# astra-vision/SceneRF

Hardware: NVIDIA H100
Metric: rays/sec (higher is better)
Workload: dtype fp32 (2 x fp16 split operands, fp32 accumulate)

## Files before the change

### scenerf_b200/csrc/mlp_tc.cu

```cuda
#include <cuda.h>
#include <cuda_fp16.h>
#include <cstdio>
#include <cstdlib>
#include <cstring>
#include <type_traits>
#include "kernels.cuh"
#include "wgmma.cuh"

namespace srf {
namespace tc {

constexpr int kTileM = 64;
constexpr int kChunkK = 64;
constexpr int kAChunkBytes = kTileM * 128;
constexpr int kBRows = 128, kBSlotBytes = kBRows * 128;
constexpr int kHiddenChunks = kHidden / kChunkK;
constexpr int kQuarters = kHidden / kBRows;
constexpr int kOutN = 16;
constexpr int kOutImgBytes = kOutN * 128;
constexpr int kThreads = 256;
constexpr int kNumBias = 8;
constexpr size_t kHeaderBytes = (size_t)kNumBias * kHidden * sizeof(float);
constexpr int kNumLayers = 11;
constexpr int kScaleSlot = 7 * kHidden + 256, kInvScaleSlot = 7 * kHidden + 257;
constexpr size_t kScratchFloats = (size_t)2 * kTileM * kHidden;
constexpr size_t kExchangeOffset = (size_t)2 * 2 * 64 * 128;

constexpr int kSmemAct = 0;
constexpr int kSmemX = kSmemAct + kHiddenChunks * kAChunkBytes;
constexpr int kSmemZ = kSmemX + kAChunkBytes;
constexpr int kRingBytes = 4 * kBSlotBytes;
constexpr int kSmemRing = kSmemZ + 2 * kAChunkBytes;
constexpr int kSmemBar = kSmemRing + 2 * kRingBytes;
constexpr int kSmemSph = kSmemBar + 2 * 4 * 8;
constexpr int kSmemMask = kSmemSph + kTileM * 4;
constexpr int kSmemTotal = kSmemMask + 16;
static_assert(kSmemTotal + 1024 <= 232448, "shared memory budget");

struct Layer { int chunks_is_kz, chunks, fresh, signal, is_out; };
__constant__ Layer kLayers[kNumLayers] = {
    {0, 1, 1, 0, 0}, {1, 0, 0, 1, 0},
    {0, 8, 1, 1, 0}, {0, 8, 1, 0, 0}, {1, 0, 0, 1, 0},
    {0, 8, 1, 1, 0}, {0, 8, 1, 0, 0}, {1, 0, 0, 1, 0},
    {0, 8, 1, 1, 0}, {0, 8, 1, 1, 0},
    {0, 8, 1, 1, 1}};

struct KernelArgs {
  const float* pts;
  const float* viewdir;
  int n, n_per, n_tiles, kz;
  const unsigned char* wblob;
  float* scratch;
  float* raw_out;
  int d_out;
  int32_t* dbg_sphere;
  int skip_zero;
  int hidden_fp16;
  const unsigned char* preproj;
  int pre_W1, pre_H1;
  int debug_layer;
  float* debug_acc;
  int* error_flag;
};

__device__ __forceinline__ uint32_t smem_u32(const void* p) { return (uint32_t)__cvta_generic_to_shared(p); }

__device__ __forceinline__ void mbar_init(uint32_t bar, uint32_t count) {
  asm volatile("mbarrier.init.shared::cta.b64 [%0], %1;" ::"r"(bar), "r"(count) : "memory");
}
__device__ __forceinline__ void mbar_arrive_expect_tx(uint32_t bar, uint32_t bytes) {
  asm volatile("mbarrier.arrive.expect_tx.shared::cta.b64 _, [%0], %1;" ::"r"(bar), "r"(bytes) : "memory");
}
__device__ __forceinline__ bool mbar_try_wait(uint32_t bar, uint32_t parity) {
  uint32_t ok;
  asm volatile(
      "{\n\t.reg .pred p;\n\t"
      "mbarrier.try_wait.parity.shared::cta.b64 p, [%1], %2;\n\t"
      "selp.u32 %0, 1, 0, p;\n\t}"
      : "=r"(ok)
      : "r"(bar), "r"(parity)
      : "memory");
  return ok != 0;
}
__device__ __noinline__ void mbar_timeout(int* error_flag, uint32_t bar, uint32_t parity) {
  if (error_flag) atomicExch(error_flag, (int)(0x40000000u | ((bar & 0xFFFFF) << 4) | (parity & 1) | ((threadIdx.x >> 5) << 24)));
  __threadfence_system();
  __trap();
}
__device__ __noinline__ void mbar_wait_spin(uint32_t bar, uint32_t parity, int* error_flag) {
  const long long t0 = clock64();
  while (!mbar_try_wait(bar, parity)) {
    if (clock64() - t0 > 4000000000LL) mbar_timeout(error_flag, bar, parity);
  }
}
__device__ __forceinline__ void mbar_wait(uint32_t bar, uint32_t parity, int* error_flag) {
  if (mbar_try_wait(bar, parity)) return;
  mbar_wait_spin(bar, parity, error_flag);
}
__device__ __forceinline__ void fence_barrier_init() { asm volatile("fence.mbarrier_init.release.cluster;" ::: "memory"); }
__device__ __forceinline__ void fence_proxy_async_smem() { asm volatile("fence.proxy.async.shared::cta;" ::: "memory"); }

__device__ __forceinline__ uint64_t l2_policy_evict_last() {
  uint64_t pol;
  asm volatile("createpolicy.fractional.L2::evict_last.b64 %0, 1.0;" : "=l"(pol));
  return pol;
}
__device__ __forceinline__ void bulk_g2s(uint32_t dst_smem, const void* src, uint32_t bytes, uint32_t bar, uint64_t policy) {
  asm volatile("cp.async.bulk.shared::cluster.global.mbarrier::complete_tx::bytes.L2::cache_hint [%0], [%1], %2, [%3], %4;"
               ::"r"(dst_smem), "l"(src), "r"(bytes), "r"(bar), "l"(policy)
               : "memory");
}
__device__ __forceinline__ void named_bar_sync(int id, int threads) {
  asm volatile("bar.sync %0, %1;" ::"r"(id), "r"(threads) : "memory");
}
__device__ __forceinline__ void sts128(uint32_t addr, uint32_t a, uint32_t b, uint32_t c, uint32_t d) {
  asm volatile("st.shared.v4.b32 [%0], {%1, %2, %3, %4};" ::"r"(addr), "r"(a), "r"(b), "r"(c), "r"(d) : "memory");
}
__device__ __forceinline__ void sts32(uint32_t addr, uint32_t a) {
  asm volatile("st.shared.b32 [%0], %1;" ::"r"(addr), "r"(a) : "memory");
}
__device__ __forceinline__ uint32_t pack_relu_half2(float lo, float hi) {
  uint32_t d;
  asm("cvt.rn.relu.f16x2.f32 %0, %1, %2;" : "=r"(d) : "f"(hi), "f"(lo));
  return d;
}
__device__ __forceinline__ uint32_t pack_half2(float lo, float hi) {
  __half2 h = __floats2half2_rn(lo, hi);
  return *reinterpret_cast<uint32_t*>(&h);
}
__device__ __forceinline__ void split_half2(float a, float b, uint32_t& hi, uint32_t& lo) {
  const __half2 h = __floats2half2_rn(a, b);
  const float2 hf = __half22float2(h);
  const __half2 l = __floats2half2_rn(a - hf.x, b - hf.y);
  hi = *reinterpret_cast<const uint32_t*>(&h);
  lo = *reinterpret_cast<const uint32_t*>(&l);
}

__device__ __forceinline__ uint32_t sw128_offset(int row, int g) { return (uint32_t)(row * 128 + ((g ^ (row & 7)) << 4)); }

__device__ __forceinline__ int layer_chunks(int l, int kz) { return kLayers[l].chunks_is_kz ? kz : kLayers[l].chunks; }
__device__ __forceinline__ bool chunk_active(int l, int c, uint64_t mask) { return !kLayers[l].chunks_is_kz || ((mask >> c) & 1ull); }

__device__ __forceinline__ uint64_t chunk_mask_for_scales(const DevParams& p, uint32_t scale_bits, int kz) {
  uint64_t m = 0;
  for (int c = 0; c < kz; ++c) {
    const int lo = c * kChunkK, hi = lo + kChunkK;
    for (int s = 0; s < kScales; ++s)
      if (((scale_bits >> s) & 1u) && p.ch_off[s] < hi && p.ch_off[s + 1] > lo) m |= 1ull << c;
  }
  return m;
}

__device__ __forceinline__ size_t chunk_image_offset(int l, int k, int kz, int parts) {
  size_t off = 0;
  for (int i = 0; i < l; ++i) off += (size_t)layer_chunks(i, kz) * (kLayers[i].is_out ? kOutImgBytes : kQuarters * kBSlotBytes);
  return (off + (size_t)k * (kLayers[l].is_out ? kOutImgBytes : kQuarters * kBSlotBytes)) * (size_t)parts;
}

struct Cursor {
  int l = 0, k = 0, j = 0;
  __device__ __forceinline__ bool normalize(int kz, uint64_t mask, int last_layer, int wg) {
    while (l <= last_layer) {
      if (l == kNumLayers - 1 && wg != 0) return false;
      if (j >= (kLayers[l].is_out ? 1 : 2)) { j = 0; ++k; }
      if (k >= layer_chunks(l, kz)) { k = 0; ++l; continue; }
      if (!chunk_active(l, k, mask)) { ++k; continue; }
      return true;
    }
    return false;
  }
};

__device__ __forceinline__ int next_active(int kz, uint64_t mask, int c) {
  for (++c; c < kz; ++c)
    if ((mask >> c) & 1ull) return c;
  return -1;
}

template <bool H16, bool SPLIT, bool PRE>
__global__ void __launch_bounds__(kThreads, 1)
point_mlp_tc_kernel(const __grid_constant__ DevParams p, const __grid_constant__ KernelArgs a) {
  extern __shared__ __align__(1024) unsigned char smem_dyn[];
  unsigned char* smem = smem_dyn + ((1024u - (smem_u32(smem_dyn) & 1023u)) & 1023u);
  const uint32_t smem_base = smem_u32(smem);
  const int tid = threadIdx.x;
  const int wg = tid >> 7, t = tid & 127, w = t >> 5, lane = tid & 31;
  constexpr int kParts = SPLIT ? 2 : 1;
  constexpr int kPts = SPLIT ? kTileM / 2 : kTileM;
  constexpr int kSlotBytes = kBSlotBytes * kParts;
  constexpr int kSlots = kRingBytes / kSlotBytes;
  const uint32_t ring = smem_base + kSmemRing + (uint32_t)wg * kRingBytes;
  auto full_bar = [&](int s) { return smem_base + kSmemBar + 8u * (uint32_t)(wg * 4 + s); };
  short2* sph_smem = reinterpret_cast<short2*>(smem + kSmemSph);
  volatile unsigned long long* mask_smem = reinterpret_cast<volatile unsigned long long*>(smem + kSmemMask);

  if (tid == 0) {
    for (int s = 0; s < 8; ++s) mbar_init(smem_base + kSmemBar + 8u * s, 1);
    fence_barrier_init();
  }
  __syncthreads();

  const int kz = a.kz;
  const int last_layer = (a.debug_layer >= 0) ? a.debug_layer : (kNumLayers - 1);
  const unsigned char* images = a.wblob + kHeaderBytes;
  const float* bias = reinterpret_cast<const float*>(a.wblob);
  float* scratch = a.scratch + (size_t)blockIdx.x * kScratchFloats;
  float* hbuf = scratch + (size_t)wg * (2 * 64 * 128);
  float* xbuf = scratch + kExchangeOffset + (size_t)wg * (2 * 64 * 64);
  const uint64_t policy = l2_policy_evict_last();

  Cursor pc;
  bool p_live = false;
  uint32_t ppos = 0, cpos = 0, done = 0;
  uint64_t mask = 0;
  auto produce = [&]() {
    if (t != 0) return;
    while (p_live && ppos < done + (uint32_t)kSlots) {
      const bool is_out = kLayers[pc.l].is_out != 0;
      const unsigned char* src = images + chunk_image_offset(pc.l, pc.k, kz, kParts) + (is_out ? 0 : (size_t)(2 * wg + pc.j) * kSlotBytes);
      const uint32_t bytes = is_out ? (uint32_t)(kOutImgBytes * kParts) : (uint32_t)kSlotBytes;
      const int s = (int)(ppos % kSlots);
      mbar_arrive_expect_tx(full_bar(s), bytes);
      bulk_g2s(ring + (uint32_t)s * kSlotBytes, src, bytes, full_bar(s), policy);
      ++ppos;
      ++pc.j;
      p_live = pc.normalize(kz, mask, last_layer, wg);
    }
  };
  float acc0[64], acc1[64], acco[8];
  auto wait_slot = [&]() -> uint32_t {
    const int s = (int)(cpos % kSlots);
    mbar_wait(full_bar(s), (cpos / kSlots) & 1u, a.error_flag);
    return ring + (uint32_t)s * kSlotBytes;
  };
  auto release1 = [&]() {
    gmma::wait<1>();
    done = cpos - 1;
    produce();
  };
  auto mma_pair = [&](uint32_t a_addr, bool fresh) {
    const uint64_t ad = gmma::desc_sw128(a_addr);
    {
      const uint32_t b = wait_slot();
      gmma::fence();
#pragma unroll
      for (int k = 0; k < 4; ++k)
#pragma unroll
        for (int part = 0; part < kParts; ++part)
          gmma::mma_f16_n128(acc0, ad + 2 * k, gmma::desc_sw128(b + part * kBSlotBytes) + 2 * k, (fresh && k == 0 && part == 0) ? 0 : 1);
      gmma::commit();
      ++cpos;
    }
    release1();
    {
      const uint32_t b = wait_slot();
      gmma::fence();
#pragma unroll
      for (int k = 0; k < 4; ++k)
#pragma unroll
        for (int part = 0; part < kParts; ++part)
          gmma::mma_f16_n128(acc1, ad + 2 * k, gmma::desc_sw128(b + part * kBSlotBytes) + 2 * k, (fresh && k == 0 && part == 0) ? 0 : 1);
      gmma::commit();
      ++cpos;
    }
  };
  auto mma_out = [&](uint32_t a_addr, bool fresh) {
    const uint64_t ad = gmma::desc_sw128(a_addr);
    const uint32_t b = wait_slot();
    gmma::fence();
#pragma unroll
    for (int k = 0; k < 4; ++k)
#pragma unroll
      for (int part = 0; part < kParts; ++part)
        gmma::mma_f16_n16(acco, ad + 2 * k, gmma::desc_sw128(b + part * kOutImgBytes) + 2 * k, (fresh && k == 0 && part == 0) ? 0 : 1);
    gmma::commit();
    ++cpos;
  };
  auto retire1 = release1;
  auto retire0 = [&]() {
    gmma::wait<0>();
    gmma::fence_regs(acc0); gmma::fence_regs(acc1); gmma::fence_regs(acco);
    done = cpos;
    produce();
  };
  auto sync_all = [&]() { named_bar_sync(1, kThreads); };

  const short2* sph_cur = sph_smem;
  const int erow0 = 16 * w + (lane >> 2);
  const int ecol = 2 * (lane & 3);

  for (int tile = blockIdx.x; tile < a.n_tiles; tile += gridDim.x) {
    const int row0 = tile * kPts;
    if (tid == 0) mask_smem[0] = 0ull;
    sync_all();
    {
      uint32_t my_scales = 0;
      if (tid < kPts) {
        const int gi = row0 + tid;
        int sx = kSphereInvalid, sy = kSphereInvalid;
        if (gi < a.n) {
          point_to_sphere(p, a.pts[(size_t)gi * 3 + 0], a.pts[(size_t)gi * 3 + 1], a.pts[(size_t)gi * 3 + 2], sx, sy);
          if (a.dbg_sphere) { a.dbg_sphere[(size_t)gi * 2 + 0] = sx; a.dbg_sphere[(size_t)gi * 2 + 1] = sy; }
        }
        sph_smem[tid] = make_short2((short)max(min(sx, 32767), -32768), (short)max(min(sy, 32767), -32768));
        if (a.skip_zero) {
#pragma unroll
          for (int s = 0; s < kScales; ++s) my_scales |= scale_taps(p, s, sx, sy).any ? (1u << s) : 0u;
        }
      }
      if (a.skip_zero && tid < ((kPts + 31) & ~31)) {
        const uint32_t wbits = __reduce_or_sync(0xffffffffu, my_scales);
        if (lane == 0) {
          const unsigned long long bits = chunk_mask_for_scales(p, wbits, kz);
          if (bits) atomicOr((unsigned long long*)mask_smem, bits);
        }
      }
    }
    sync_all();
    mask = PRE ? 0ull : (a.skip_zero ? mask_smem[0] : ~0ull);
    pc = Cursor();
    p_live = pc.normalize(kz, mask, last_layer, wg);
    produce();

    const unsigned char* pre_row[2] = {nullptr, nullptr};
    if constexpr (PRE) {
#pragma unroll
      for (int hh = 0; hh < 2; ++hh) {
        const short2 sp = sph_cur[(erow0 + 8 * hh) % kPts];
        const bool in = sp.x >= 0 && sp.x < a.pre_W1 && sp.y >= 0 && sp.y < a.pre_H1;
        const size_t ridx = in ? (size_t)sp.y * a.pre_W1 + sp.x : (size_t)a.pre_W1 * a.pre_H1;
        pre_row[hh] = a.preproj + ridx * (size_t)(SRF_NUM_BLOCKS * kHidden * (SPLIT ? 4 : 2));
      }
    }

    if (tid < 2 * kPts) {
      const bool first = tid < kPts;
      const int xrow = first ? tid : tid - kPts;
      const int gi = row0 + xrow;
      const uint32_t slot_addr = smem_base + kSmemX;
      float qx = 0.f, qy = 0.f, qz = 0.f;
      if (gi < a.n) { qx = a.pts[(size_t)gi * 3 + 0]; qy = a.pts[(size_t)gi * 3 + 1]; qz = a.pts[(size_t)gi * 3 + 2]; }
      const float kPi = 3.14159274101257324f, kHalfPi = 1.57079637050628662f;
      auto sel3 = [](int i, float v0, float v1, float v2) { return i == 0 ? v0 : (i == 1 ? v1 : v2); };
      auto xval = [&](int idx, const float* vd) -> float {
        if (gi >= a.n) return 0.0f;
        if (idx < 3) return sel3(idx, qx, qy, qz);
        if (idx < 3 + 36) {
          const int j = idx - 3, fp = j / 3, cc = j - 3 * fp;
          float arg = fmul(sel3(cc, qx, qy, qz), kPi * (float)(1 << (fp >> 1)));
          if (fp & 1) arg = fadd(kHalfPi, arg);
          return sinf(arg);
        }
        if (idx < kDX) return sel3(idx - 39, vd[0], vd[1], vd[2]);
        return 0.0f;
      };
      float vd[3] = {0.f, 0.f, 0.f};
      if (!first && gi < a.n) {
        const float* vp = a.viewdir + (size_t)(gi / a.n_per) * 3;
        vd[0] = vp[0]; vd[1] = vp[1]; vd[2] = vp[2];
      }
      const int g_end = first ? 3 : 8;
#pragma unroll 1
      for (int g = first ? 0 : 3; g < g_end; ++g) {
        float v[8];
#pragma unroll
        for (int j = 0; j < 8; ++j) v[j] = xval(8 * g + j, vd);
        if constexpr (SPLIT) {
          uint32_t hi[4], lo[4];
#pragma unroll
          for (int j = 0; j < 4; ++j) split_half2(v[2 * j], v[2 * j + 1], hi[j], lo[j]);
          sts128(slot_addr + sw128_offset(xrow, g), hi[0], hi[1], hi[2], hi[3]);
          sts128(slot_addr + sw128_offset(xrow + kPts, g), lo[0], lo[1], lo[2], lo[3]);
        } else {
          sts128(slot_addr + sw128_offset(xrow, g), pack_half2(v[0], v[1]), pack_half2(v[2], v[3]), pack_half2(v[4], v[5]),
                 pack_half2(v[6], v[7]));
        }
      }
    }
    fence_proxy_async_smem();
    sync_all();

    constexpr int kItems = kPts / 32;
    int cur_scale = -1;
    int t_off[kItems];
    uint32_t t_ok[kItems];
    float t_w[kItems], t_n[kItems];
    int dxo = 0, dyo = 0;
    auto gather = [&](int c, uint32_t zaddr) {
      const int g = tid & 7;
      const int ch = c * kChunkK + g * 8;
      auto emit_vals = [&](int row, const float (&v)[8]) {
        if constexpr (SPLIT) {
          uint32_t hi[4], lo[4];
#pragma unroll
          for (int j = 0; j < 4; ++j) split_half2(v[2 * j], v[2 * j + 1], hi[j], lo[j]);
          sts128(zaddr + sw128_offset(row, g), hi[0], hi[1], hi[2], hi[3]);
          sts128(zaddr + sw128_offset(row + kPts, g), lo[0], lo[1], lo[2], lo[3]);
        } else {
          sts128(zaddr + sw128_offset(row, g), pack_half2(v[0], v[1]), pack_half2(v[2], v[3]), pack_half2(v[4], v[5]), pack_half2(v[6], v[7]));
        }
      };
      int s = -1;
#pragma unroll
      for (int i = 0; i < kScales; ++i)
        if (ch >= p.ch_off[i] && ch < p.ch_off[i + 1]) s = i;
      if (s >= 0 && s != cur_scale) {
        dxo = p.C[s]; dyo = p.W[s] * p.C[s];
#pragma unroll
        for (int i = 0; i < kItems; ++i) {
          const short2 sp16 = sph_cur[(tid >> 3) + 32 * i];
          const Taps tp = scale_taps(p, s, sp16.x, sp16.y);
          t_ok[i] = (tp.off[0] >= 0 ? 1u : 0u) | (tp.off[1] >= 0 ? 2u : 0u) | (tp.off[2] >= 0 ? 4u : 0u) | (tp.off[3] >= 0 ? 8u : 0u);
          int o0 = 0;
          if (tp.off[0] >= 0) o0 = tp.off[0];
          else if (tp.off[1] >= 0) o0 = tp.off[1] - dxo;
          else if (tp.off[2] >= 0) o0 = tp.off[2] - dyo;
          else if (tp.off[3] >= 0) o0 = tp.off[3] - dxo - dyo;
          t_off[i] = o0;
          t_w[i] = tp.fx; t_n[i] = tp.fy;
        }
        cur_scale = s;
      }
      const char* fbytes = (s >= 0) ? reinterpret_cast<const char*>(p.feat[s]) : nullptr;
      const int ch_in = (s >= 0) ? ch - p.ch_off[s] : 0;
      const bool f16 = p.feat_fp16 != 0;
#pragma unroll
      for (int u = 0; u < kItems; ++u) {
        const int row = (tid >> 3) + 32 * u;
        float acc[8];
        const uint32_t ok = (s >= 0) ? t_ok[u] : 0u;
        if (!ok) {
#pragma unroll
          for (int e = 0; e < 8; ++e) acc[e] = 0.0f;
          emit_vals(row, acc);
          continue;
        }
        const float wx = t_w[u], ny = t_n[u];
        const float e_ = fsub(1.0f, wx), so = fsub(1.0f, ny);
        const float tw4[4] = {fmul(so, e_), fmul(so, wx), fmul(ny, e_), fmul(ny, wx)};
        float v[4][8];
#pragma unroll
        for (int tp = 0; tp < 4; ++tp) {
          if ((ok >> tp) & 1u) {
            const size_t eidx = (size_t)(ch_in + t_off[u] + (tp & 1) * dxo + (tp >> 1) * dyo);
            if (f16) {
              const uint4 raw = __ldg(reinterpret_cast<const uint4*>(fbytes + eidx * 2));
              const uint32_t rw[4] = {raw.x, raw.y, raw.z, raw.w};
#pragma unroll
              for (int q = 0; q < 4; ++q) {
                const float2 f = __half22float2(*reinterpret_cast<const __half2*>(&rw[q]));
                v[tp][2 * q] = f.x; v[tp][2 * q + 1] = f.y;
              }
            } else {
              const float4* src = reinterpret_cast<const float4*>(fbytes + eidx * 4);
              const float4 a0 = __ldg(src), a1 = __ldg(src + 1);
              v[tp][0] = a0.x; v[tp][1] = a0.y; v[tp][2] = a0.z; v[tp][3] = a0.w;
              v[tp][4] = a1.x; v[tp][5] = a1.y; v[tp][6] = a1.z; v[tp][7] = a1.w;
            }
          } else {
#pragma unroll
            for (int e = 0; e < 8; ++e) v[tp][e] = 0.0f;
          }
        }
#pragma unroll
        for (int e = 0; e < 8; ++e) {
          acc[e] = fmul(v[0][e], tw4[0]);
#pragma unroll
          for (int tp = 1; tp < 4; ++tp) acc[e] = fadd(acc[e], fmul(v[tp][e], tw4[tp]));
        }
        emit_vals(row, acc);
      }
    };
    auto zpass = [&]() {
      cur_scale = -1;
      int c = next_active(kz, mask, -1);
      if (c < 0) return;
      gather(c, smem_base + kSmemZ);
      fence_proxy_async_smem();
      sync_all();
      for (int zi = 0; c >= 0; ++zi) {
        const int cn = next_active(kz, mask, c);
        mma_pair(smem_base + kSmemZ + (uint32_t)(zi & 1) * kAChunkBytes, false);
        if (cn >= 0) gather(cn, smem_base + kSmemZ + (uint32_t)((zi + 1) & 1) * kAChunkBytes);
        retire0();
        fence_proxy_async_smem();
        sync_all();
        c = cn;
      }
    };

    auto epilogue = [&](auto use_h_c, auto write_h_c, auto use_p_c, int bias_idx) __attribute__((always_inline)) {
      constexpr bool USE_H = decltype(use_h_c)::value, WRITE_H = decltype(write_h_c)::value, USE_P = decltype(use_p_c)::value;
      if constexpr (SPLIT) {
        if (t >= 64) {
#pragma unroll
          for (int i = 0; i < 64; ++i) { xbuf[i * 64 + (t - 64)] = acc0[i]; xbuf[(64 + i) * 64 + (t - 64)] = acc1[i]; }
        }
        named_bar_sync(2 + wg, 128);
        if (t >= 64) return;
      }
      [[maybe_unused]] const float inv_scale = SPLIT ? __ldg(bias + kInvScaleSlot) : 1.0f;
      auto finish = [&](float (&acc)[64], int j) __attribute__((always_inline)) {
#pragma unroll
        for (int i2 = 0; i2 < 32; ++i2) {
          const int i = 2 * i2, hh = i2 & 1;
          const int row = erow0 + 8 * hh;
          const int col = 256 * wg + 128 * j + 8 * (i2 >> 1) + ecol;
          float r0 = acc[i], r1 = acc[i + 1];
          if constexpr (SPLIT) {
            const float p0 = xbuf[(j * 64 + i) * 64 + t], p1 = xbuf[(j * 64 + i + 1) * 64 + t];
            r0 = (r0 + p0) * inv_scale; r1 = (r1 + p1) * inv_scale;
          }
          if constexpr (!USE_P) {
            const float2 bb = __ldg(reinterpret_cast<const float2*>(bias + (size_t)bias_idx * kHidden + col));
            r0 += bb.x; r1 += bb.y;
          }
          [[maybe_unused]] float2* hp = reinterpret_cast<float2*>(hbuf) + (size_t)(j * 32 + i2) * 128 + t;
          [[maybe_unused]] __half2* hp16 = reinterpret_cast<__half2*>(hbuf) + (size_t)(j * 32 + i2) * 128 + t;
          if constexpr (USE_H) {
            if constexpr (H16) { const float2 f = __half22float2(*hp16); r0 += f.x; r1 += f.y; }
            else { const float2 f = *hp; r0 += f.x; r1 += f.y; }
          }
          if constexpr (USE_P) {
            if constexpr (SPLIT) {
              const float2 f = __ldg(reinterpret_cast<const float2*>(pre_row[hh] + ((size_t)bias_idx * kHidden + col) * 4));
              r0 += f.x; r1 += f.y;
            } else {
              const float2 f = __half22float2(__ldg(reinterpret_cast<const __half2*>(pre_row[hh] + ((size_t)bias_idx * kHidden + col) * 2)));
              r0 += f.x; r1 += f.y;
            }
          }
          if constexpr (WRITE_H) {
            if constexpr (H16) *hp16 = __floats2half2_rn(r0, r1);
            else *hp = make_float2(r0, r1);
          }
          const uint32_t addr = smem_base + kSmemAct + (uint32_t)(col >> 6) * kAChunkBytes;
          const uint32_t inrow = (uint32_t)((((col & 63) >> 3) ^ (row & 7)) << 4) + (uint32_t)((col & 7) * 2);
          if constexpr (SPLIT) {
            uint32_t hi, lo;
            split_half2(fmaxf(r0, 0.0f), fmaxf(r1, 0.0f), hi, lo);
            sts32(addr + (uint32_t)row * 128 + inrow, hi);
            sts32(addr + (uint32_t)(row + kPts) * 128 + inrow, lo);
          } else {
            sts32(addr + (uint32_t)row * 128 + inrow, pack_relu_half2(r0, r1));
          }
        }
      };
      finish(acc0, 0);
      finish(acc1, 1);
    };
    auto epi = [&](auto use_h_c, auto write_h_c, auto use_p_c, int bias_idx) __attribute__((always_inline)) {
      retire0();
      sync_all();
      epilogue(use_h_c, write_h_c, use_p_c, bias_idx);
      fence_proxy_async_smem();
      sync_all();
    };
    auto dump_acc = [&](bool out) {
      retire0();
      if (out && wg != 0) return;
#pragma unroll
      for (int hh = 0; hh < 2; ++hh) {
        float* dst = a.debug_acc + ((size_t)tile * kTileM + erow0 + 8 * hh) * kHidden;
        if (out) {
#pragma unroll
          for (int c8 = 0; c8 < 2; ++c8) { dst[8 * c8 + ecol] = acco[4 * c8 + 2 * hh]; dst[8 * c8 + ecol + 1] = acco[4 * c8 + 2 * hh + 1]; }
        } else {
#pragma unroll
          for (int c8 = 0; c8 < 16; ++c8) {
            const int col = 256 * wg + 8 * c8 + ecol;
            dst[col] = acc0[4 * c8 + 2 * hh]; dst[col + 1] = acc0[4 * c8 + 2 * hh + 1];
            dst[col + 128] = acc1[4 * c8 + 2 * hh]; dst[col + 129] = acc1[4 * c8 + 2 * hh + 1];
          }
        }
      }
    };

    using T = std::true_type;
    using F = std::false_type;
    using P = std::integral_constant<bool, PRE>;
    mma_pair(smem_base + kSmemX, true);
    retire1();
    if (!PRE) zpass();
    if (a.debug_layer == 1) { dump_acc(false); continue; }
    bool stop = false;
    for (int b = 0; b < SRF_NUM_BLOCKS; ++b) {
      if (b == 0) epi(F{}, T{}, P{}, b);
      else epi(T{}, T{}, P{}, b);
#pragma unroll 1
      for (int k = 0; k < kHiddenChunks; ++k) { mma_pair(smem_base + kSmemAct + (uint32_t)k * kAChunkBytes, k == 0); retire1(); }
      if (a.debug_layer == 2 + 3 * b) { dump_acc(false); stop = true; break; }
      epi(F{}, F{}, F{}, 3 + b);
#pragma unroll 1
      for (int k = 0; k < kHiddenChunks; ++k) { mma_pair(smem_base + kSmemAct + (uint32_t)k * kAChunkBytes, k == 0); retire1(); }
      if (b < SRF_NUM_BLOCKS - 1) {
        if (!PRE) zpass();
        if (a.debug_layer == 4 + 3 * b) { dump_acc(false); stop = true; break; }
      } else if (a.debug_layer == 9) { dump_acc(false); stop = true; break; }
    }
    if (stop) continue;
    epi(T{}, F{}, F{}, 6);
    if (wg == 0) {
#pragma unroll 1
      for (int k = 0; k < kHiddenChunks; ++k) { mma_out(smem_base + kSmemAct + (uint32_t)k * kAChunkBytes, k == 0); retire1(); }
      if (a.debug_layer == 10) { dump_acc(true); continue; }
      retire0();
      const float* bo = bias + (size_t)7 * kHidden;
      if constexpr (SPLIT) {
        if (t >= 64) {
#pragma unroll
          for (int i = 0; i < 8; ++i) xbuf[i * 64 + (t - 64)] = acco[i];
        }
        named_bar_sync(2, 128);
      }
      if (!SPLIT || t < 64) {
        const float inv_scale = SPLIT ? __ldg(bias + kInvScaleSlot) : 1.0f;
#pragma unroll
        for (int i = 0; i < 8; ++i) {
          const int row = erow0 + 8 * ((i >> 1) & 1);
          const int col = 8 * (i >> 2) + ecol + (i & 1);
          float v = acco[i];
          if constexpr (SPLIT) v = (v + xbuf[i * 64 + t]) * inv_scale;
          const int gi = row0 + row;
          if (row < kPts && gi < a.n && col < a.d_out) a.raw_out[(size_t)gi * a.d_out + col] = v + __ldg(bo + col);
        }
      }
    }
  }
}

struct PackArgs {
  srf_mlp_weights w;
  int kz;
  int parts;
};

__device__ __forceinline__ const float* layer_weight(const srf_mlp_weights& w, int l, int& K) {
  K = kHidden;
  switch (l) {
    case 0: K = kDX; return w.lin_in_w;
    case 1: K = w.d_latent; return w.lin_z_w[0];
    case 2: return w.fc0_w[0];
    case 3: return w.fc1_w[0];
    case 4: K = w.d_latent; return w.lin_z_w[1];
    case 5: return w.fc0_w[1];
    case 6: return w.fc1_w[1];
    case 7: K = w.d_latent; return w.lin_z_w[2];
    case 8: return w.fc0_w[2];
    case 9: return w.fc1_w[2];
    default: return w.lin_out_w;
  }
}

__global__ void weight_absmax_kernel(const __grid_constant__ PackArgs pa, unsigned int* __restrict__ max_bits) {
  float m = 0.0f;
  for (int l = 0; l < kNumLayers; ++l) {
    int K;
    const float* W = layer_weight(pa.w, l, K);
    const size_t n = (size_t)(l == kNumLayers - 1 ? pa.w.d_out : kHidden) * K;
    for (size_t i = (size_t)blockIdx.x * blockDim.x + threadIdx.x; i < n; i += (size_t)gridDim.x * blockDim.x) m = fmaxf(m, fabsf(W[i]));
  }
#pragma unroll
  for (int o = 16; o > 0; o >>= 1) m = fmaxf(m, __shfl_xor_sync(0xffffffffu, m, o));
  if ((threadIdx.x & 31) == 0) atomicMax(max_bits, __float_as_uint(m));
}
__global__ void weight_scale_kernel(const unsigned int* __restrict__ max_bits, float* __restrict__ hdr, int split) {
  float scale = 1.0f;
  if (split) {
    const float m = __uint_as_float(*max_bits);
    int e = 0;
    if (m > 0.0f && isfinite(m)) { frexpf(m, &e); e = 14 - e; }
    e = max(-40, min(40, e));
    scale = ldexpf(1.0f, e);
  }
  hdr[kScaleSlot] = scale;
  hdr[kInvScaleSlot] = 1.0f / scale;
}

__global__ void pack_images_kernel(const __grid_constant__ PackArgs pa, const float* __restrict__ hdr, unsigned char* __restrict__ images,
                                   size_t n_granules) {
  const size_t gid = (size_t)blockIdx.x * blockDim.x + threadIdx.x;
  if (gid >= n_granules) return;
  size_t byte = gid * 16;
  const int parts = pa.parts;
  const float scale = hdr[kScaleSlot];
  int l = 0;
  size_t off = 0;
  for (; l < kNumLayers; ++l) {
    const size_t sz = (size_t)layer_chunks(l, pa.kz) * (kLayers[l].is_out ? kOutImgBytes : kQuarters * kBSlotBytes) * parts;
    if (byte < off + sz) break;
    off += sz;
  }
  const size_t rel = byte - off;
  const bool is_out = kLayers[l].is_out;
  const size_t img_bytes = is_out ? kOutImgBytes : kBSlotBytes;
  const size_t chunk_bytes = (is_out ? 1 : kQuarters) * img_bytes * parts;
  const int c = (int)(rel / chunk_bytes);
  const size_t in_chunk = rel % chunk_bytes;
  const int img = (int)(in_chunk / img_bytes);
  const int q = img / parts, part = img % parts;
  const size_t in_img = in_chunk % img_bytes;
  const int row = (int)(in_img / 128);
  const int gpos = (int)((in_img % 128) / 16);
  const int g = gpos ^ (row & 7);
  const int n = q * kBRows + row;
  int K;
  const float* W = layer_weight(pa.w, l, K);
  const int n_rows = is_out ? pa.w.d_out : kHidden;
  __align__(16) __half hv[8];
#pragma unroll
  for (int j = 0; j < 8; ++j) {
    const int k = c * kChunkK + g * 8 + j;
    const float v = ((n < n_rows && k < K) ? W[(size_t)n * K + k] : 0.0f) * scale;
    const __half hi = __float2half_rn(v);
    hv[j] = part == 0 ? hi : __float2half_rn(v - __half2float(hi));
  }
  *reinterpret_cast<uint4*>(images + byte) = *reinterpret_cast<const uint4*>(hv);
}

__global__ void pack_header_kernel(const __grid_constant__ PackArgs pa, float* __restrict__ hdr) {
  const int j = blockIdx.x * blockDim.x + threadIdx.x;
  if (j >= kHidden) return;
  const srf_mlp_weights& w = pa.w;
  hdr[0 * kHidden + j] = w.lin_in_b[j] + w.lin_z_b[0][j];
  hdr[1 * kHidden + j] = w.fc1_b[0][j] + w.lin_z_b[1][j];
  hdr[2 * kHidden + j] = w.fc1_b[1][j] + w.lin_z_b[2][j];
  hdr[3 * kHidden + j] = w.fc0_b[0][j];
  hdr[4 * kHidden + j] = w.fc0_b[1][j];
  hdr[5 * kHidden + j] = w.fc0_b[2][j];
  hdr[6 * kHidden + j] = w.fc1_b[2][j];
  hdr[7 * kHidden + j] = (j < w.d_out) ? w.lin_out_b[j] : 0.0f;
}

static size_t images_bytes(int kz, int parts = 1) {
  size_t b = 0;
  const int chunks[kNumLayers] = {1, kz, 8, 8, kz, 8, 8, kz, 8, 8, 8};
  for (int l = 0; l < kNumLayers; ++l) b += (size_t)chunks[l] * (l == kNumLayers - 1 ? kOutImgBytes : kQuarters * kBSlotBytes);
  return b * (size_t)parts;
}

}

static inline int kz_of(int d_latent) { return (d_latent + tc::kChunkK - 1) / tc::kChunkK; }

size_t tc_weights_bytes(int d_out, int d_latent, int split) {
  (void)d_out;
  return tc::kHeaderBytes + tc::images_bytes(kz_of(d_latent), split ? 2 : 1) + 256;
}

int pack_weights_tc(const srf_mlp_weights& w, void* dst, size_t bytes, int split, cudaStream_t st) {
  const int kz = kz_of(w.d_latent);
  if (kz > 64 || w.d_out < 1 || w.d_out > tc::kOutN || (w.d_latent % 8)) return 1;
  const size_t need = tc_weights_bytes(w.d_out, w.d_latent, split);
  if (bytes < need) return 1;
  tc::PackArgs pa;
  pa.w = w;
  pa.kz = kz;
  pa.parts = split ? 2 : 1;
  float* hdr = reinterpret_cast<float*>(dst);
  unsigned int* max_bits = reinterpret_cast<unsigned int*>(reinterpret_cast<unsigned char*>(dst) + need - 4);
  tc::pack_header_kernel<<<(kHidden + 127) / 128, 128, 0, st>>>(pa, hdr);
  if (split) {
    cudaMemsetAsync(max_bits, 0, 4, st);
    tc::weight_absmax_kernel<<<296, 256, 0, st>>>(pa, max_bits);
  }
  tc::weight_scale_kernel<<<1, 1, 0, st>>>(max_bits, hdr, split ? 1 : 0);
  const size_t n_gran = tc::images_bytes(kz, pa.parts) / 16;
  tc::pack_images_kernel<<<(unsigned)((n_gran + 255) / 256), 256, 0, st>>>(
      pa, hdr, reinterpret_cast<unsigned char*>(dst) + tc::kHeaderBytes, n_gran);
  return 0;
}

static int* g_wd_host = nullptr;
static int* g_wd_dev = nullptr;
int tc_watchdog_flag() { return g_wd_host ? *g_wd_host : 0; }

static int num_sms() { return device_sm_count(); }

using TcKernelFn = void (*)(const DevParams, const tc::KernelArgs);
constexpr int kNumTcKernels = 6;
static TcKernelFn tc_kernel_at(int i) {
  static const TcKernelFn table[kNumTcKernels] = {
      tc::point_mlp_tc_kernel<false, false, false>, tc::point_mlp_tc_kernel<true, false, false>, tc::point_mlp_tc_kernel<false, true, false>,
      tc::point_mlp_tc_kernel<false, false, true>,  tc::point_mlp_tc_kernel<true, false, true>,  tc::point_mlp_tc_kernel<false, true, true>};
  return table[i];
}
static TcKernelFn tc_kernel(bool h16, bool split, bool pre) { return tc_kernel_at((split ? 2 : (h16 ? 1 : 0)) + (pre ? 3 : 0)); }

constexpr int kMaxTcCtas = 256;
size_t tc_workspace_bytes(int d_latent, int n_points) {
  (void)d_latent; (void)n_points;
  return (size_t)kMaxTcCtas * tc::kScratchFloats * sizeof(float) + 256;
}

int run_point_mlp_tc_debug(const DevParams& p, const srf_mlp_weights& w, const float* pts, const float* viewdir, int n,
                           int n_per, float* raw_out, int32_t* dbg_sphere, int flags, void* workspace, size_t ws_bytes,
                           int debug_layer, float* debug_acc, cudaStream_t st) {
  if (ws_bytes < tc_workspace_bytes(p.d_latent, n)) return -1;
  if (debug_layer >= 0 && !(debug_layer < tc::kNumLayers && debug_layer != 0 && debug_layer != 3 && debug_layer != 6))
    return -2;
  const size_t smem = tc::kSmemTotal + 1024;
  static bool attr_set = false;
  if (!attr_set) {
    for (int i = 0; i < kNumTcKernels; ++i) cudaFuncSetAttribute(tc_kernel_at(i), cudaFuncAttributeMaxDynamicSharedMemorySize, (int)smem);
    attr_set = true;
  }
  const bool split = (flags & kTcFlagSplit) != 0;
  const int tile_pts = split ? tc::kTileM / 2 : tc::kTileM;
  tc::KernelArgs a;
  a.pts = pts; a.viewdir = viewdir; a.n = n; a.n_per = n_per;
  a.n_tiles = (n + tile_pts - 1) / tile_pts;
  a.kz = kz_of(p.d_latent);
  a.wblob = reinterpret_cast<const unsigned char*>(split ? w.tc_split_packed : w.tc_packed);
  if (!a.wblob) return -3;
  a.scratch = reinterpret_cast<float*>(workspace);
  a.raw_out = raw_out; a.d_out = w.d_out; a.dbg_sphere = dbg_sphere;
  a.skip_zero = (flags & SRF_FLAG_SKIP_ZERO_CHUNKS) ? 1 : 0;
  a.hidden_fp16 = (!split && (flags & SRF_FLAG_HIDDEN_FP16)) ? 1 : 0;
  a.preproj = nullptr; a.pre_W1 = p.sphere_W + 1; a.pre_H1 = p.sphere_H + 1;
  if ((flags & kTcFlagPreproj) && p.preproj && (p.preproj_fp16 != 0) == !split) {
    a.preproj = reinterpret_cast<const unsigned char*>(p.preproj);
    a.skip_zero = 0;
  }
  a.debug_layer = debug_layer; a.debug_acc = debug_acc;
  if (!g_wd_host) {
    if (cudaHostAlloc(reinterpret_cast<void**>(&g_wd_host), sizeof(int), cudaHostAllocMapped) == cudaSuccess) {
      *g_wd_host = 0;
      cudaHostGetDevicePointer(reinterpret_cast<void**>(&g_wd_dev), g_wd_host, 0);
    }
  }
  a.error_flag = g_wd_dev;
  int grid = a.n_tiles < num_sms() ? a.n_tiles : num_sms();
  if (grid > kMaxTcCtas) grid = kMaxTcCtas;
  if (grid < 1) return 0;
  tc_kernel(a.hidden_fp16 != 0, split, a.preproj != nullptr)<<<grid, tc::kThreads, smem, st>>>(p, a);
  return 1;
}

int run_point_mlp_tc(const DevParams& p, const srf_mlp_weights& w, const float* pts, const float* viewdir, int n,
                     int n_per, float* raw_out, int32_t* dbg_sphere, int flags, void* workspace, size_t ws_bytes,
                     cudaStream_t st) {
  return run_point_mlp_tc_debug(p, w, pts, viewdir, n, n_per, raw_out, dbg_sphere, flags, workspace, ws_bytes, -1,
                                nullptr, st);
}

}
```

Before: 62680.

## Restructure split-fp16 MMA to full 64-row tiles with separate hi/lo operand chunks

In split mode, the tile previously packed hi and lo halves as rows of a 64-row A tile, so only 32 points were processed per tile and partial sums were exchanged through a global scratch buffer. Now each tile holds 64 points, hi and lo A chunks are stored side by side in shared memory, and the three cross terms (hi*hi, lo*hi, hi*lo) are issued as separate wgmma calls into one accumulator. The weight ring is changed to stream single hi or lo B images per slot, with fewer slots in split mode. Latent-pass accumulation is periodically flushed to scratch in groups to limit fp16-split error growth. The goal is to double the points per tile and drop the half-warpgroup exchange and reduction, at the cost of extra MMAs per chunk and a smaller ring.

```diff
diff --git a/scenerf_b200/csrc/mlp_tc.cu b/scenerf_b200/csrc/mlp_tc.cu
--- a/scenerf_b200/csrc/mlp_tc.cu
+++ b/scenerf_b200/csrc/mlp_tc.cu
@@ -24,18 +24,24 @@
 constexpr int kNumLayers = 11;
 constexpr int kScaleSlot = 7 * kHidden + 256, kInvScaleSlot = 7 * kHidden + 257;
 constexpr size_t kScratchFloats = (size_t)2 * kTileM * kHidden;
-constexpr size_t kExchangeOffset = (size_t)2 * 2 * 64 * 128;
-
-constexpr int kSmemAct = 0;
-constexpr int kSmemX = kSmemAct + kHiddenChunks * kAChunkBytes;
-constexpr int kSmemZ = kSmemX + kAChunkBytes;
-constexpr int kRingBytes = 4 * kBSlotBytes;
-constexpr int kSmemRing = kSmemZ + 2 * kAChunkBytes;
-constexpr int kSmemBar = kSmemRing + 2 * kRingBytes;
-constexpr int kSmemSph = kSmemBar + 2 * 4 * 8;
-constexpr int kSmemMask = kSmemSph + kTileM * 4;
-constexpr int kSmemTotal = kSmemMask + 16;
-static_assert(kSmemTotal + 1024 <= 232448, "shared memory budget");
+constexpr int kZGroup = 13;
+
+template <bool SPLIT>
+struct Smem {
+  static constexpr int kAStride = (SPLIT ? 2 : 1) * kAChunkBytes;
+  static constexpr int kAct = 0;
+  static constexpr int kX = SPLIT ? kAct : kAct + kHiddenChunks * kAStride;
+  static constexpr int kZ = SPLIT ? kAct + kAStride : kX + kAChunkBytes;
+  static constexpr int kSlots = SPLIT ? 3 : 4;
+  static constexpr int kRingBytes = kSlots * kBSlotBytes;
+  static constexpr int kRing = SPLIT ? kAct + kHiddenChunks * kAStride : kZ + 2 * kAChunkBytes;
+  static constexpr int kBar = kRing + 2 * kRingBytes;
+  static constexpr int kSph = kBar + 2 * 4 * 8;
+  static constexpr int kMask = kSph + kTileM * 4;
+  static constexpr int kTotal = kMask + 16;
+  static_assert(kTotal + 1024 <= 232448, "shared memory budget");
+  static_assert(!SPLIT || (kZ >= kX + kAStride && kZ + 2 * kAStride <= kAct + (kHiddenChunks - 1) * kAStride), "latent pairs");
+};
 
 struct Layer { int chunks_is_kz, chunks, fresh, signal, is_out; };
 __constant__ Layer kLayers[kNumLayers] = {
@@ -159,10 +165,10 @@
 
 struct Cursor {
   int l = 0, k = 0, j = 0;
-  __device__ __forceinline__ bool normalize(int kz, uint64_t mask, int last_layer, int wg) {
+  __device__ __forceinline__ bool normalize(int kz, uint64_t mask, int last_layer, int wg, int imgs) {
     while (l <= last_layer) {
       if (l == kNumLayers - 1 && wg != 0) return false;
-      if (j >= (kLayers[l].is_out ? 1 : 2)) { j = 0; ++k; }
+      if (j >= (kLayers[l].is_out ? 1 : imgs)) { j = 0; ++k; }
       if (k >= layer_chunks(l, kz)) { k = 0; ++l; continue; }
       if (!chunk_active(l, k, mask)) { ++k; continue; }
       return true;
@@ -185,17 +191,16 @@
   const uint32_t smem_base = smem_u32(smem);
   const int tid = threadIdx.x;
   const int wg = tid >> 7, t = tid & 127, w = t >> 5, lane = tid & 31;
+  using L = Smem<SPLIT>;
   constexpr int kParts = SPLIT ? 2 : 1;
-  constexpr int kPts = SPLIT ? kTileM / 2 : kTileM;
-  constexpr int kSlotBytes = kBSlotBytes * kParts;
-  constexpr int kSlots = kRingBytes / kSlotBytes;
-  const uint32_t ring = smem_base + kSmemRing + (uint32_t)wg * kRingBytes;
-  auto full_bar = [&](int s) { return smem_base + kSmemBar + 8u * (uint32_t)(wg * 4 + s); };
-  short2* sph_smem = reinterpret_cast<short2*>(smem + kSmemSph);
-  volatile unsigned long long* mask_smem = reinterpret_cast<volatile unsigned long long*>(smem + kSmemMask);
+  constexpr int kSlots = L::kSlots;
+  const uint32_t ring = smem_base + L::kRing + (uint32_t)wg * L::kRingBytes;
+  auto full_bar = [&](int s) { return smem_base + L::kBar + 8u * (uint32_t)(wg * 4 + s); };
+  short2* sph_smem = reinterpret_cast<short2*>(smem + L::kSph);
+  volatile unsigned long long* mask_smem = reinterpret_cast<volatile unsigned long long*>(smem + L::kMask);
 
   if (tid == 0) {
-    for (int s = 0; s < 8; ++s) mbar_init(smem_base + kSmemBar + 8u * s, 1);
+    for (int s = 0; s < 8; ++s) mbar_init(smem_base + L::kBar + 8u * s, 1);
     fence_barrier_init();
   }
   __syncthreads();
@@ -206,7 +211,7 @@
   const float* bias = reinterpret_cast<const float*>(a.wblob);
   float* scratch = a.scratch + (size_t)blockIdx.x * kScratchFloats;
   float* hbuf = scratch + (size_t)wg * (2 * 64 * 128);
-  float* xbuf = scratch + kExchangeOffset + (size_t)wg * (2 * 64 * 64);
+  float* zsum = scratch + (size_t)kTileM * kHidden + (size_t)wg * (2 * 64 * 128);
   const uint64_t policy = l2_policy_evict_last();
 
   Cursor pc;
@@ -217,62 +222,70 @@
     if (t != 0) return;
     while (p_live && ppos < done + (uint32_t)kSlots) {
       const bool is_out = kLayers[pc.l].is_out != 0;
-      const unsigned char* src = images + chunk_image_offset(pc.l, pc.k, kz, kParts) + (is_out ? 0 : (size_t)(2 * wg + pc.j) * kSlotBytes);
-      const uint32_t bytes = is_out ? (uint32_t)(kOutImgBytes * kParts) : (uint32_t)kSlotBytes;
+      const unsigned char* src = images + chunk_image_offset(pc.l, pc.k, kz, kParts) + (is_out ? 0 : (size_t)(2 * kParts * wg + pc.j) * kBSlotBytes);
+      const uint32_t bytes = is_out ? (uint32_t)(kOutImgBytes * kParts) : (uint32_t)kBSlotBytes;
       const int s = (int)(ppos % kSlots);
       mbar_arrive_expect_tx(full_bar(s), bytes);
-      bulk_g2s(ring + (uint32_t)s * kSlotBytes, src, bytes, full_bar(s), policy);
+      bulk_g2s(ring + (uint32_t)s * kBSlotBytes, src, bytes, full_bar(s), policy);
       ++ppos;
       ++pc.j;
-      p_live = pc.normalize(kz, mask, last_layer, wg);
+      p_live = pc.normalize(kz, mask, last_layer, wg, 2 * kParts);
     }
   };
   float acc0[64], acc1[64], acco[8];
   auto wait_slot = [&]() -> uint32_t {
     const int s = (int)(cpos % kSlots);
     mbar_wait(full_bar(s), (cpos / kSlots) & 1u, a.error_flag);
-    return ring + (uint32_t)s * kSlotBytes;
+    return ring + (uint32_t)s * kBSlotBytes;
   };
   auto release1 = [&]() {
     gmma::wait<1>();
     done = cpos - 1;
     produce();
   };
-  auto mma_pair = [&](uint32_t a_addr, bool fresh) {
+  constexpr uint64_t kLoDesc = kAChunkBytes >> 4;
+  auto mma_quarter = [&](float (&acc)[64], uint32_t a_addr, bool fresh) __attribute__((always_inline)) {
     const uint64_t ad = gmma::desc_sw128(a_addr);
     {
-      const uint32_t b = wait_slot();
+      const uint64_t bd = gmma::desc_sw128(wait_slot());
       gmma::fence();
 #pragma unroll
-      for (int k = 0; k < 4; ++k)
-#pragma unroll
-        for (int part = 0; part < kParts; ++part)
-          gmma::mma_f16_n128(acc0, ad + 2 * k, gmma::desc_sw128(b + part * kBSlotBytes) + 2 * k, (fresh && k == 0 && part == 0) ? 0 : 1);
+      for (int k = 0; k < 4; ++k) {
+        gmma::mma_f16_n128(acc, ad + 2 * k, bd + 2 * k, (fresh && k == 0) ? 0 : 1);
+        if constexpr (SPLIT) gmma::mma_f16_n128(acc, ad + kLoDesc + 2 * k, bd + 2 * k, 1);
+      }
       gmma::commit();
       ++cpos;
     }
-    release1();
-    {
-      const uint32_t b = wait_slot();
+    if constexpr (SPLIT) {
+      release1();
+      const uint64_t bd = gmma::desc_sw128(wait_slot());
       gmma::fence();
 #pragma unroll
-      for (int k = 0; k < 4; ++k)
-#pragma unroll
-        for (int part = 0; part < kParts; ++part)
-          gmma::mma_f16_n128(acc1, ad + 2 * k, gmma::desc_sw128(b + part * kBSlotBytes) + 2 * k, (fresh && k == 0 && part == 0) ? 0 : 1);
+      for (int k = 0; k < 4; ++k) gmma::mma_f16_n128(acc, ad + 2 * k, bd + 2 * k, 1);
       gmma::commit();
       ++cpos;
     }
+  };
+  auto mma_pair = [&](uint32_t a_addr, bool fresh) {
+    mma_quarter(acc0, a_addr, fresh);
+    release1();
+    mma_quarter(acc1, a_addr, fresh);
   };
   auto mma_out = [&](uint32_t a_addr, bool fresh) {
     const uint64_t ad = gmma::desc_sw128(a_addr);
     const uint32_t b = wait_slot();
+    const uint64_t bd = gmma::desc_sw128(b);
     gmma::fence();
 #pragma unroll
-    for (int k = 0; k < 4; ++k)
-#pragma unroll
-      for (int part = 0; part < kParts; ++part)
-        gmma::mma_f16_n16(acco, ad + 2 * k, gmma::desc_sw128(b + part * kOutImgBytes) + 2 * k, (fresh && k == 0 && part == 0) ? 0 : 1);
+    for (int k = 0; k < 4; ++k) {
+      gmma::mma_f16_n16(acco, ad + 2 * k, bd + 2 * k, (fresh && k == 0) ? 0 : 1);
+      if constexpr (SPLIT) gmma::mma_f16_n16(acco, ad + kLoDesc + 2 * k, bd + 2 * k, 1);
+    }
+    if constexpr (SPLIT) {
+#pragma unroll
+      for (int k = 0; k < 4; ++k) gmma::mma_f16_n16(acco, ad + 2 * k, bd + (kOutImgBytes >> 4) + 2 * k, 1);
+    }
     gmma::commit();
     ++cpos;
   };
@@ -290,12 +303,12 @@
   const int ecol = 2 * (lane & 3);
 
   for (int tile = blockIdx.x; tile < a.n_tiles; tile += gridDim.x) {
-    const int row0 = tile * kPts;
+    const int row0 = tile * kTileM;
     if (tid == 0) mask_smem[0] = 0ull;
     sync_all();
     {
       uint32_t my_scales = 0;
-      if (tid < kPts) {
+      if (tid < kTileM) {
         const int gi = row0 + tid;
         int sx = kSphereInvalid, sy = kSphereInvalid;
         if (gi < a.n) {
@@ -308,7 +321,7 @@
           for (int s = 0; s < kScales; ++s) my_scales |= scale_taps(p, s, sx, sy).any ? (1u << s) : 0u;
         }
       }
-      if (a.skip_zero && tid < ((kPts + 31) & ~31)) {
+      if (a.skip_zero && tid < kTileM) {
         const uint32_t wbits = __reduce_or_sync(0xffffffffu, my_scales);
         if (lane == 0) {
           const unsigned long long bits = chunk_mask_for_scales(p, wbits, kz);
@@ -319,25 +332,25 @@
     sync_all();
     mask = PRE ? 0ull : (a.skip_zero ? mask_smem[0] : ~0ull);
     pc = Cursor();
-    p_live = pc.normalize(kz, mask, last_layer, wg);
+    p_live = pc.normalize(kz, mask, last_layer, wg, 2 * kParts);
     produce();
 
     const unsigned char* pre_row[2] = {nullptr, nullptr};
     if constexpr (PRE) {
 #pragma unroll
       for (int hh = 0; hh < 2; ++hh) {
-        const short2 sp = sph_cur[(erow0 + 8 * hh) % kPts];
+        const short2 sp = sph_cur[erow0 + 8 * hh];
         const bool in = sp.x >= 0 && sp.x < a.pre_W1 && sp.y >= 0 && sp.y < a.pre_H1;
         const size_t ridx = in ? (size_t)sp.y * a.pre_W1 + sp.x : (size_t)a.pre_W1 * a.pre_H1;
         pre_row[hh] = a.preproj + ridx * (size_t)(SRF_NUM_BLOCKS * kHidden * (SPLIT ? 4 : 2));
       }
     }
 
-    if (tid < 2 * kPts) {
-      const bool first = tid < kPts;
-      const int xrow = first ? tid : tid - kPts;
+    if (tid < 2 * kTileM) {
+      const bool first = tid < kTileM;
+      const int xrow = first ? tid : tid - kTileM;
       const int gi = row0 + xrow;
-      const uint32_t slot_addr = smem_base + kSmemX;
+      const uint32_t slot_addr = smem_base + L::kX;
       float qx = 0.f, qy = 0.f, qz = 0.f;
       if (gi < a.n) { qx = a.pts[(size_t)gi * 3 + 0]; qy = a.pts[(size_t)gi * 3 + 1]; qz = a.pts[(size_t)gi * 3 + 2]; }
       const float kPi = 3.14159274101257324f, kHalfPi = 1.57079637050628662f;
@@ -370,7 +383,7 @@
 #pragma unroll
           for (int j = 0; j < 4; ++j) split_half2(v[2 * j], v[2 * j + 1], hi[j], lo[j]);
           sts128(slot_addr + sw128_offset(xrow, g), hi[0], hi[1], hi[2], hi[3]);
-          sts128(slot_addr + sw128_offset(xrow + kPts, g), lo[0], lo[1], lo[2], lo[3]);
+          sts128(slot_addr + kAChunkBytes + sw128_offset(xrow, g), lo[0], lo[1], lo[2], lo[3]);
         } else {
           sts128(slot_addr + sw128_offset(xrow, g), pack_half2(v[0], v[1]), pack_half2(v[2], v[3]), pack_half2(v[4], v[5]),
                  pack_half2(v[6], v[7]));
@@ -380,7 +393,7 @@
     fence_proxy_async_smem();
     sync_all();
 
-    constexpr int kItems = kPts / 32;
+    constexpr int kItems = kTileM / 32;
     int cur_scale = -1;
     int t_off[kItems];
     uint32_t t_ok[kItems];
@@ -395,7 +408,7 @@
 #pragma unroll
           for (int j = 0; j < 4; ++j) split_half2(v[2 * j], v[2 * j + 1], hi[j], lo[j]);
           sts128(zaddr + sw128_offset(row, g), hi[0], hi[1], hi[2], hi[3]);
-          sts128(zaddr + sw128_offset(row + kPts, g), lo[0], lo[1], lo[2], lo[3]);
+          sts128(zaddr + kAChunkBytes + sw128_offset(row, g), lo[0], lo[1], lo[2], lo[3]);
         } else {
           sts128(zaddr + sw128_offset(row, g), pack_half2(v[0], v[1]), pack_half2(v[2], v[3]), pack_half2(v[4], v[5]), pack_half2(v[6], v[7]));
         }
@@ -475,14 +488,29 @@
       cur_scale = -1;
       int c = next_active(kz, mask, -1);
       if (c < 0) return;
-      gather(c, smem_base + kSmemZ);
+      if constexpr (SPLIT) {
+        retire0();
+#pragma unroll
+        for (int i = 0; i < 64; ++i) { zsum[i * 128 + t] = acc0[i]; zsum[(64 + i) * 128 + t] = acc1[i]; }
+        sync_all();
+      }
+      gather(c, smem_base + L::kZ);
       fence_proxy_async_smem();
       sync_all();
       for (int zi = 0; c >= 0; ++zi) {
         const int cn = next_active(kz, mask, c);
-        mma_pair(smem_base + kSmemZ + (uint32_t)(zi & 1) * kAChunkBytes, false);
-        if (cn >= 0) gather(cn, smem_base + kSmemZ + (uint32_t)((zi + 1) & 1) * kAChunkBytes);
+        mma_pair(smem_base + L::kZ + (uint32_t)(zi & 1) * L::kAStride, SPLIT && zi % kZGroup == 0);
+        if (cn >= 0) gather(cn, smem_base + L::kZ + (uint32_t)((zi + 1) & 1) * L::kAStride);
         retire0();
+        if constexpr (SPLIT) {
+          if (cn < 0) {
+#pragma unroll
+            for (int i = 0; i < 64; ++i) { acc0[i] += zsum[i * 128 + t]; acc1[i] += zsum[(64 + i) * 128 + t]; }
+          } else if ((zi + 1) % kZGroup == 0) {
+#pragma unroll
+            for (int i = 0; i < 64; ++i) { zsum[i * 128 + t] += acc0[i]; zsum[(64 + i) * 128 + t] += acc1[i]; }
+          }
+        }
         fence_proxy_async_smem();
         sync_all();
         c = cn;
@@ -491,15 +519,9 @@
 
     auto epilogue = [&](auto use_h_c, auto write_h_c, auto use_p_c, int bias_idx) __attribute__((always_inline)) {
       constexpr bool USE_H = decltype(use_h_c)::value, WRITE_H = decltype(write_h_c)::value, USE_P = decltype(use_p_c)::value;
-      if constexpr (SPLIT) {
-        if (t >= 64) {
-#pragma unroll
-          for (int i = 0; i < 64; ++i) { xbuf[i * 64 + (t - 64)] = acc0[i]; xbuf[(64 + i) * 64 + (t - 64)] = acc1[i]; }
-        }
-        named_bar_sync(2 + wg, 128);
-        if (t >= 64) return;
-      }
       [[maybe_unused]] const float inv_scale = SPLIT ? __ldg(bias + kInvScaleSlot) : 1.0f;
+      uint32_t act_base = smem_base + L::kAct;
+      if constexpr (SPLIT) asm volatile("mov.b32 %0, %0;" : "+r"(act_base));
       auto finish = [&](float (&acc)[64], int j) __attribute__((always_inline)) {
 #pragma unroll
         for (int i2 = 0; i2 < 32; ++i2) {
@@ -507,10 +529,7 @@
           const int row = erow0 + 8 * hh;
           const int col = 256 * wg + 128 * j + 8 * (i2 >> 1) + ecol;
           float r0 = acc[i], r1 = acc[i + 1];
-          if constexpr (SPLIT) {
-            const float p0 = xbuf[(j * 64 + i) * 64 + t], p1 = xbuf[(j * 64 + i + 1) * 64 + t];
-            r0 = (r0 + p0) * inv_scale; r1 = (r1 + p1) * inv_scale;
-          }
+          if constexpr (SPLIT) { r0 *= inv_scale; r1 *= inv_scale; }
           if constexpr (!USE_P) {
             const float2 bb = __ldg(reinterpret_cast<const float2*>(bias + (size_t)bias_idx * kHidden + col));
             r0 += bb.x; r1 += bb.y;
@@ -534,13 +553,13 @@
             if constexpr (H16) *hp16 = __floats2half2_rn(r0, r1);
             else *hp = make_float2(r0, r1);
           }
-          const uint32_t addr = smem_base + kSmemAct + (uint32_t)(col >> 6) * kAChunkBytes;
+          const uint32_t addr = act_base + (uint32_t)(col >> 6) * L::kAStride;
           const uint32_t inrow = (uint32_t)((((col & 63) >> 3) ^ (row & 7)) << 4) + (uint32_t)((col & 7) * 2);
           if constexpr (SPLIT) {
             uint32_t hi, lo;
             split_half2(fmaxf(r0, 0.0f), fmaxf(r1, 0.0f), hi, lo);
             sts32(addr + (uint32_t)row * 128 + inrow, hi);
-            sts32(addr + (uint32_t)(row + kPts) * 128 + inrow, lo);
+            sts32(addr + kAChunkBytes + (uint32_t)row * 128 + inrow, lo);
           } else {
             sts32(addr + (uint32_t)row * 128 + inrow, pack_relu_half2(r0, r1));
           }
@@ -561,7 +580,9 @@
       if (out && wg != 0) return;
 #pragma unroll
       for (int hh = 0; hh < 2; ++hh) {
-        float* dst = a.debug_acc + ((size_t)tile * kTileM + erow0 + 8 * hh) * kHidden;
+        const int pt = tile * kTileM + erow0 + 8 * hh;
+        if (SPLIT && (pt & ~31) >= a.n) continue;
+        float* dst = a.debug_acc + (SPLIT ? (size_t)(pt >> 5) * 64 + (pt & 31) : (size_t)pt) * kHidden;
         if (out) {
 #pragma unroll
           for (int c8 = 0; c8 < 2; ++c8) { dst[8 * c8 + ecol] = acco[4 * c8 + 2 * hh]; dst[8 * c8 + ecol + 1] = acco[4 * c8 + 2 * hh + 1]; }
@@ -579,7 +600,7 @@
     using T = std::true_type;
     using F = std::false_type;
     using P = std::integral_constant<bool, PRE>;
-    mma_pair(smem_base + kSmemX, true);
+    mma_pair(smem_base + L::kX, true);
     retire1();
     if (!PRE) zpass();
     if (a.debug_layer == 1) { dump_acc(false); continue; }
@@ -588,11 +609,11 @@
       if (b == 0) epi(F{}, T{}, P{}, b);
       else epi(T{}, T{}, P{}, b);
 #pragma unroll 1
-      for (int k = 0; k < kHiddenChunks; ++k) { mma_pair(smem_base + kSmemAct + (uint32_t)k * kAChunkBytes, k == 0); retire1(); }
+      for (int k = 0; k < kHiddenChunks; ++k) { mma_pair(smem_base + L::kAct + (uint32_t)k * L::kAStride, k == 0); retire1(); }
       if (a.debug_layer == 2 + 3 * b) { dump_acc(false); stop = true; break; }
       epi(F{}, F{}, F{}, 3 + b);
 #pragma unroll 1
-      for (int k = 0; k < kHiddenChunks; ++k) { mma_pair(smem_base + kSmemAct + (uint32_t)k * kAChunkBytes, k == 0); retire1(); }
+      for (int k = 0; k < kHiddenChunks; ++k) { mma_pair(smem_base + L::kAct + (uint32_t)k * L::kAStride, k == 0); retire1(); }
       if (b < SRF_NUM_BLOCKS - 1) {
         if (!PRE) zpass();
         if (a.debug_layer == 4 + 3 * b) { dump_acc(false); stop = true; break; }
@@ -602,28 +623,19 @@
     epi(T{}, F{}, F{}, 6);
     if (wg == 0) {
 #pragma unroll 1
-      for (int k = 0; k < kHiddenChunks; ++k) { mma_out(smem_base + kSmemAct + (uint32_t)k * kAChunkBytes, k == 0); retire1(); }
+      for (int k = 0; k < kHiddenChunks; ++k) { mma_out(smem_base + L::kAct + (uint32_t)k * L::kAStride, k == 0); retire1(); }
       if (a.debug_layer == 10) { dump_acc(true); continue; }
       retire0();
       const float* bo = bias + (size_t)7 * kHidden;
-      if constexpr (SPLIT) {
-        if (t >= 64) {
-#pragma unroll
-          for (int i = 0; i < 8; ++i) xbuf[i * 64 + (t - 64)] = acco[i];
-        }
-        named_bar_sync(2, 128);
-      }
-      if (!SPLIT || t < 64) {
-        const float inv_scale = SPLIT ? __ldg(bias + kInvScaleSlot) : 1.0f;
-#pragma unroll
-        for (int i = 0; i < 8; ++i) {
-          const int row = erow0 + 8 * ((i >> 1) & 1);
-          const int col = 8 * (i >> 2) + ecol + (i & 1);
-          float v = acco[i];
-          if constexpr (SPLIT) v = (v + xbuf[i * 64 + t]) * inv_scale;
-          const int gi = row0 + row;
-          if (row < kPts && gi < a.n && col < a.d_out) a.raw_out[(size_t)gi * a.d_out + col] = v + __ldg(bo + col);
-        }
+      [[maybe_unused]] const float inv_scale = SPLIT ? __ldg(bias + kInvScaleSlot) : 1.0f;
+#pragma unroll
+      for (int i = 0; i < 8; ++i) {
+        const int row = erow0 + 8 * ((i >> 1) & 1);
+        const int col = 8 * (i >> 2) + ecol + (i & 1);
+        float v = acco[i];
+        if constexpr (SPLIT) v *= inv_scale;
+        const int gi = row0 + row;
+        if (gi < a.n && col < a.d_out) a.raw_out[(size_t)gi * a.d_out + col] = v + __ldg(bo + col);
       }
     }
   }
@@ -786,6 +798,7 @@
   return table[i];
 }
 static TcKernelFn tc_kernel(bool h16, bool split, bool pre) { return tc_kernel_at((split ? 2 : (h16 ? 1 : 0)) + (pre ? 3 : 0)); }
+static size_t tc_smem_bytes(bool split) { return (split ? tc::Smem<true>::kTotal : tc::Smem<false>::kTotal) + 1024; }
 
 constexpr int kMaxTcCtas = 256;
 size_t tc_workspace_bytes(int d_latent, int n_points) {
@@ -799,17 +812,17 @@
   if (ws_bytes < tc_workspace_bytes(p.d_latent, n)) return -1;
   if (debug_layer >= 0 && !(debug_layer < tc::kNumLayers && debug_layer != 0 && debug_layer != 3 && debug_layer != 6))
     return -2;
-  const size_t smem = tc::kSmemTotal + 1024;
   static bool attr_set = false;
   if (!attr_set) {
-    for (int i = 0; i < kNumTcKernels; ++i) cudaFuncSetAttribute(tc_kernel_at(i), cudaFuncAttributeMaxDynamicSharedMemorySize, (int)smem);
+    for (int i = 0; i < kNumTcKernels; ++i)
+      cudaFuncSetAttribute(tc_kernel_at(i), cudaFuncAttributeMaxDynamicSharedMemorySize, (int)tc_smem_bytes(i % 3 == 2));
     attr_set = true;
   }
   const bool split = (flags & kTcFlagSplit) != 0;
-  const int tile_pts = split ? tc::kTileM / 2 : tc::kTileM;
+  const size_t smem = tc_smem_bytes(split);
   tc::KernelArgs a;
   a.pts = pts; a.viewdir = viewdir; a.n = n; a.n_per = n_per;
-  a.n_tiles = (n + tile_pts - 1) / tile_pts;
+  a.n_tiles = (n + tc::kTileM - 1) / tc::kTileM;
   a.kz = kz_of(p.d_latent);
   a.wblob = reinterpret_cast<const unsigned char*>(split ? w.tc_split_packed : w.tc_packed);
   if (!a.wblob) return -3;
```

Result: faster. 84280, median of 6 (+34.5%).
